# johannah/drqv2

Hardware: NVIDIA B200
Metric: DrQ-v2 updates/sec at batch 256 (higher is better)
Workload: dtype bf16

## Files before the change

drqv2_b200/_bf16.py:

```python
from __future__ import annotations

import ctypes as C

import torch

from . import _lib
from ._lib import (GEMM_KK, GEMM_KMN, GEMM_MNMN, PLB, REPR_DIM, TB_ACT, TB_W, TEPI_F32, TEPI_MASK_BF16,
                   TEPI_RELU_BF16, TEPI_TRUNK_DGRAD, TEPI_TRUNK_WGRAD, WB_SLACK, call)

F32, BF = 4, 2


def _stream():
    return torch.cuda.current_stream().cuda_stream


def _ceil(n, m):
    return (n + m - 1) // m * m


def splitk_for(ctas_per_split, K=REPR_DIM, target_blocks=148):
    s0 = max(1, min(target_blocks // max(1, ctas_per_split), K // 128))
    chunk = -(-K // s0)
    chunk = -(-chunk // 128) * 128
# ... 439 lines not shown
                     ws.metrics.data_ptr() + F32 * 6, xA.ptr(), xA.units, Fd, 0)])
    if split_q:
        twin_q_layers(agent, bw, bw.x, 1, 1, B)
        beside.join()
        twin_q_heads(agent, bw, 2, B)
    else:
        twin_q_fwd(agent, bw, bw.x, 2, B)
    q = bw.q4.data_ptr()
    c1, c2, dc1, dc2 = bw.c1, bw.c2, bw.dc1, bw.dc2
    w0, w2, xC = st.q0, st.q2, bw.x
    U, HS = c1.units, c1.stride
    call("drq_q_head_bwd_loss_bf16", 1, q, q + F32 * 2 * B, ws.reward.data_ptr(), ws.discount.data_ptr(),
         ws.target_q.data_ptr(), ws.metrics.data_ptr(), c2.ptr(), U, HS, pc("Q1.4.weight"), dc2.ptr(),
         gc("Q1.4.weight"), gc("Q1.4.bias"), B, H, qs_f, s)
    with beside:
        gemm(dc2.ptr(), U, c1.ptr(), U, GEMM_MNMN, gc("Q1.2.weight"), H, H, H, B, TEPI_F32, batch=2,
             strides=_strides((HS, HS, qs_f, 0, 0)), bn=128)
    gemm(dc2.ptr(), U, w2.ptr(), w2.units, GEMM_KMN, dc1.ptr(), U, B, H, H, TEPI_MASK_BF16, mask=c1.ptr(), units_mask=U,
         batch=2, strides=_strides((HS, w2.stride, HS, 0, HS)))
    with beside:
        gemm(dc1.ptr(), U, xC.ptr(0), xC.units, GEMM_MNMN, gc("Q1.0.weight"), Fd + A, H, Fd + A, B, TEPI_F32, batch=2,
             strides=_strides((HS, 0, qs_f, 0, 0)))
    PS = B * (Fd + A)
    gemm(dc1.ptr(), U, w0.ptr(), w0.units, GEMM_KMN, bw.dxf.data_ptr(), Fd + A, B, Fd, H, TEPI_F32, batch=2,
         splitk=bw.SX, strides=_strides((HS, w0.stride, PS, 0, 0), split=2 * PS))
    call("drq_ln_tanh_bwd", bw.dxf.data_ptr(), Fd + A, ws.xC.data_ptr(), Fd + A, ws.xhatC.data_ptr(),
         ws.rstdC.data_ptr(), pc("trunk.1.weight"), ws.dz.data_ptr(), None, None,
         bw.dz.ptr(), bw.dz.units, B, Fd, 2 * bw.SX, PS, s)
    with beside:
        gemm(bw.dz.ptr(), bw.dz.units, feat.ptr(), feat.units, GEMM_MNMN, gc("trunk.0.weight"), REPR_DIM, Fd, REPR_DIM, B,
             TEPI_TRUNK_WGRAD, bn=128)
        colsum_multi([ColsumJob(dc2.ptr(0), U, gc("Q1.2.bias"), B, H, 1, 0), ColsumJob(dc2.ptr(1), U, gc("Q2.2.bias"), B, H, 1, 0),
                      ColsumJob(dc1.ptr(0), U, gc("Q1.0.bias"), B, H, 1, 0), ColsumJob(dc1.ptr(1), U, gc("Q2.0.bias"), B, H, 1, 0),
                      ColsumJob(ws.dz.data_ptr(), Fd, gc("trunk.0.bias"), B, Fd, 0, 0),
                      ColsumJob(ws.dz.data_ptr() + F32 * B * Fd, Fd, gc("trunk.1.weight"), B, Fd, 0, 0, ws.xhatC.data_ptr()),
                      ColsumJob(ws.dz.data_ptr() + F32 * B * Fd, Fd, gc("trunk.1.bias"), B, Fd, 0, 0)])
    d = [t.data_ptr() for t in bw.dpre]
    acts = [t.data_ptr() for t in bw.acts]
    ge = lambda k: agent._g("encoder", k)
    if not encoder_grad:
        beside.join()
        agent._sync_grads("critic")
        st.step_critic()
        return
    gemm(bw.dz.ptr(), bw.dz.units, st.trunk_ptr(st.CRITIC), st.trunk.units, GEMM_KMN, d[3], bw.cs_d, B, REPR_DIM, Fd,
         TEPI_TRUNK_DGRAD, mask=feat.ptr(), units_mask=feat.units, bn=128)
    def encoder_backward():
        s2 = _stream()
# ... 209 lines not shown
```

drqv2_b200/_lib.py:

```python
from __future__ import annotations

import ctypes as C
import os
import pathlib

_HERE = pathlib.Path(__file__).resolve().parent
LIB_PATH = _HERE / "csrc" / "libdrqv2_b200.so"

P = C.c_void_p
I = C.c_int
L = C.c_int64
U = C.c_uint64
F = C.c_float

SIGNATURES = {
    "drq_ring_gather_nstep": [P, P, P, P, L, I, I, I, P, P, I, I, F, P, P, P, P, P, P],
    "drq_ring_sample": [P, P, I, U, P, P, P, I, P],
    "drq_rng_update_draws": [U, P, I, P, P, P, P, I, I, P],
    "drq_ring_sample_step": [P, P, I, U, P, P, P, I, P],
    "drq_update_prologue": [P, I, P, P, U, P, I, P, P, P, P, I, I, P],
    "drq_update_prologue_ring": [P, I, P, P, U, P, I, P, P, P, P, I, I, P, P, P, P, P],
    "drq_update_prologue_ring_part": [P, I, P, P, U, P, I, P, P, P, P, I, I, P, P, P, P, I, P],
    "drq_conv1_fwd_bf16_ring": [P, I, P, P, P, I, I, P],
    "drq_conv1_wgrad_bf16_ring": [P, I, P, P, P, P, P, I, I, P],
    "drq_rng_normal_f32": [U, P, P, I, P],
    "drq_counter_advance": [P, P],
    "drq_scalars_fetch": [P, I, P, P, P],
    "drq_random_shift_f32": [P, P, P, I, I, I, I, I, P],
    "drq_conv1_fwd_f32": [P, P, P, P, P, I, I, I, P],
    "drq_conv1_wgrad_f32": [P, P, P, P, P, P, I, I, I, P],
    "drq_conv3x3_fwd_f32": [P, P, P, P, I, I, I, P],
    "drq_conv3x3_dgrad_f32": [P, P, P, P, I, I, P],
    "drq_conv3x3_wgrad_f32": [P, P, P, P, P, I, I, P],
    "drq_pack_conv_w_bf16": [P, P, P, P],
    "drq_conv3x3_fwd_bf16": [P, P, P, P, I, I, I, L, I, I, P],
    "drq_conv3x3_dgrad_bf16": [P, P, P, I, P, I, I, P],
    "drq_conv3x3_wgrad_bf16": [P, I, P, P, P, P, I, I, P],
    "drq_pack_conv1_w_bf16": [P, P, P, I, P],
    "drq_conv1_fwd_bf16": [P, P, P, P, I, I, I, P],
    "drq_conv1_wgrad_bf16": [P, P, P, P, P, P, I, I, I, P],
    "drq_gemm_bf16": [P, I, P, I, I, P, L, I, P, P, I, I, I, I, I, I, I, I, P, I, I, P],
    "drq_set_pdl": [I],
    "drq_set_sm_limit": [I],
    "drq_set_gemm_small": [I],
    "drq_set_conv4x1": [I],
    "drq_set_conv1_planes": [I],
    "drq_debug_gemm_stamps": [P],
    "drq_debug_opt_min_blocks": [I],
    "drq_debug_conv_stamps": [P],
    "drq_debug_trap_note": [P],
    "drq_debug_force_timeout": [P],
    "drq_debug_conv4x1_stamps": [P],
    "drq_debug_conv1_stamps": [P],
    "drq_pack_multi": [P, I, P],
    "drq_conv_wgrad_reduce_multi": [P, I, P],
    "drq_colsum_multi": [P, I, P],
    "drq_pack_linear_tb": [P, P, I, I, P],
    "drq_pack_trunk_tb": [P, P, I, P],
    "drq_pack_features_tb": [P, P, I, P],
    "drq_gemm_f32": [P, L, L, P, L, L, P, L, P, P, L, I, I, I, I, I, I, L, L, L, L, L, I, P],
    "drq_colsum_f32": [P, L, P, I, I, I, L, L, P],
    "drq_ln_tanh_fwd": [P, I, L, P, P, P, P, L, P, P, P, L, I, I, F, P],
    "drq_ln_tanh_fwd_multi": [P, I, I, I, F, P],
    "drq_ln_tanh_bwd": [P, L, P, L, P, P, P, P, P, P, P, L, I, I, I, L, P],
    "drq_actor_sample": [P, P, P, F, P, L, P, P, P, L, I, I, I, P],
    "drq_policy_head_fwd_bf16": [P, L, P, P, P, I, I, I, P, I, P, F, P, P],
    "drq_actor_sample_bwd": [P, L, P, P, P, L, I, I, I, L, P],
# ... 35 lines not shown


def lib():
    global _lib
    if _lib is None:
        if not LIB_PATH.exists():
            raise ImportError(
                f"{LIB_PATH} is missing: build the CUDA extension first (make -C {LIB_PATH.parent}). "
                "drqv2_b200 has no CPU or PyTorch fallback.")
        h = C.CDLL(str(LIB_PATH))
        for name, args in SIGNATURES.items():
            fn = getattr(h, name)
            fn.argtypes, fn.restype = args, I
        for name, (res, args) in SPECIAL.items():
            fn = getattr(h, name)
            fn.argtypes, fn.restype = args, res
        if h.drq_abi_version() != 1:
            raise ImportError("libdrqv2_b200.so ABI version mismatch")
        h.drq_set_pdl(int(os.environ.get("DRQV2_B200_PDL", "0")))
        if os.environ.get("DRQV2_B200_OPT_MINB"):
            h.drq_debug_opt_min_blocks(int(os.environ["DRQV2_B200_OPT_MINB"]))
        if os.environ.get("DRQV2_B200_CONV4X1"):
            h.drq_set_conv4x1(int(os.environ["DRQV2_B200_CONV4X1"]))
        if os.environ.get("DRQV2_B200_CONV1_PLANES"):
            h.drq_set_conv1_planes(int(os.environ["DRQV2_B200_CONV1_PLANES"]))
        _lib = h
    return _lib


def exported_symbols():
    return list(SIGNATURES) + list(SPECIAL)


def call(name, *args):
    rc = getattr(lib(), name)(*args)
    if rc != 0:
        raise DrqError(f"{name} failed ({rc}): {lib().drq_last_error().decode()}")


def ptr(t):
    return None if t is None else t.data_ptr()
```

drqv2_b200/csrc/common.cuh:

```cuda
#pragma once
#include <cuda_runtime.h>
#include <stdint.h>

#include "../../include/drqv2_b200.h"

namespace drq {

void set_error(const char* fmt, ...);

int check_launch(const char* what);

int ensure_smem(const void* kernel, size_t bytes, const char* what);

inline cudaStream_t as_stream(void* s) { return reinterpret_cast<cudaStream_t>(s); }

void* tensor_map_encoder();

extern int g_pdl;
extern int g_pdl_once;
extern int g_sm_limit;
inline int sm_budget() { return g_sm_limit; }
__device__ __forceinline__ void pdl_trigger() {
#ifdef DRQ_PDL_ENTRY_TRIGGER
    asm volatile("griddepcontrol.launch_dependents;" ::: "memory");
#endif
}
__device__ __forceinline__ void pdl_release() { asm volatile("griddepcontrol.launch_dependents;" ::: "memory"); }
__device__ __forceinline__ void pdl_wait() { asm volatile("griddepcontrol.wait;" ::: "memory"); }

template <typename... P, typename... A>
inline void launch_k(void (*kernel)(P...), dim3 grid, dim3 block, size_t smem, cudaStream_t stream, A&&... args) {
    cudaLaunchConfig_t cfg{};
    cfg.gridDim = grid; cfg.blockDim = block; cfg.dynamicSmemBytes = smem; cfg.stream = stream;
    cudaLaunchAttribute attr[1];
    attr[0].id = cudaLaunchAttributeProgrammaticStreamSerialization;
    attr[0].val.programmaticStreamSerializationAllowed = 1;
    cfg.attrs = attr; cfg.numAttrs = (g_pdl == 1 || (g_pdl == 2 && g_pdl_once)) ? 1 : 0;
    g_pdl_once = 0;
    cudaLaunchKernelEx(&cfg, kernel, static_cast<P>(args)...);
}

constexpr int kImg = DRQ_IMG;
constexpr int kPW = DRQ_PW;
constexpr int kPlane = DRQ_PLANE;
constexpr int kCh = DRQ_CONV_CH;

__device__ __forceinline__ int clampi(int v, int lo, int hi) { return v < lo ? lo : (v > hi ? hi : v); }

__device__ __forceinline__ float warp_sum(float v) {
#pragma unroll
    for (int o = 16; o > 0; o >>= 1) v += __shfl_xor_sync(0xffffffffu, v, o);
    return v;
}

struct Philox {
    static constexpr uint32_t kM0 = 0xD2511F53u, kM1 = 0xCD9E8D57u;
    static constexpr uint32_t kW0 = 0x9E3779B9u, kW1 = 0xBB67AE85u;
    __host__ __device__ static inline void round(uint32_t (&c)[4], uint32_t k0, uint32_t k1) {
        uint64_t p0 = (uint64_t)kM0 * c[0], p1 = (uint64_t)kM1 * c[2];
        uint32_t h0 = (uint32_t)(p0 >> 32), l0 = (uint32_t)p0;
        uint32_t h1 = (uint32_t)(p1 >> 32), l1 = (uint32_t)p1;
        uint32_t n0 = h1 ^ c[1] ^ k0, n2 = h0 ^ c[3] ^ k1;
// ... 26 lines not shown
```

drqv2_b200/csrc/gemm_tc.cu:

```cuda
#include "pack.cuh"

namespace drq {

DRQ_TRAP_NOTE_HOOK(trap_note_gemm)

using namespace tc;

constexpr int GT_BM = 128, GT_THREADS = 192;
constexpr int RA = DRQ_TB_ACT, RW = DRQ_TB_W;
constexpr int MODE_KK = DRQ_GEMM_KK, MODE_KMN = DRQ_GEMM_KMN, MODE_MNMN = DRQ_GEMM_MNMN;

struct GemmTcArgs {
    const __nv_bfloat16* A; int units_a;
    const __nv_bfloat16* B; int units_b;
    int M, N, K;
    int batch_inner; long long bs[11];
    int splitk, k_chunk, nz;
    int grid3d;
    int accumulate;
    float* Cf; __nv_bfloat16* Cb; long long ldc;
    int n_store;
    const float* bias;
    const __nv_bfloat16* mask; int units_mask;
    long long* stamps;
};

static long long* g_stamps = nullptr;
#ifdef DRQ_STAMPS
#define GT_STAMP(i) do { if (g.stamps && (blockIdx.x | blockIdx.y | blockIdx.z) == 0) g.stamps[i] = clock64(); } while (0)
#else
#define GT_STAMP(i) do { } while (0)
#endif

template <int MODE, int BN, int EPI, int SMALL = 0>
struct GemmCfg {
    static constexpr int BK = MODE == MODE_MNMN ? RA : 64;
    static constexpr int A_BYTES = MODE == MODE_MNMN ? 16 * RA * 16 : 8 * RA * 16;
    static constexpr int B_BYTES = MODE == MODE_KK ? 8 * BN * 16 : (MODE == MODE_KMN ? (BN / 8) * RW * 16 : (BN / 8) * RA * 16);
    static constexpr int STAGE = A_BYTES + B_BYTES;
    static constexpr bool XPOSE = EPI == DRQ_TEPI_F32 || EPI == DRQ_TEPI_TRUNK_WGRAD;
    static constexpr int XP_FLOATS = EPI == DRQ_TEPI_TRUNK_WGRAD ? 32 * (BN + 1) : (XPOSE ? 32 * 33 : 0);
    static constexpr int EPI_BYTES = 2 * BN * 4 + 4 * XP_FLOATS * 4;
    static constexpr int BUDGET = 196 * 1024 - EPI_BYTES;
    static constexpr int STAGES = SMALL ? 2 : (BUDGET / STAGE > 6 ? 6 : BUDGET / STAGE);
    static constexpr int ACC = 2;
    static constexpr int B_COPIES = (MODE == MODE_KK && BN == 128) ? 2 : 1;
    static constexpr size_t SMEM = (size_t)STAGES * STAGE + EPI_BYTES + (2 * STAGES + 2 * ACC) * 8 + 16;
};

struct TileInfo {
    int m0, n0, k_begin, k_end;
    long long off_a, off_b, off_c, off_bias, off_mask;
};
template <int BN>
__device__ __forceinline__ TileInfo tile_info(const GemmTcArgs& g, int t, int nt, int mt) {
    TileInfo ti;
    int in, im, z;
    if (g.grid3d) {
        in = blockIdx.x; im = blockIdx.y; z = blockIdx.z;
    } else {
        in = t; im = 0; z = 0;
        if (nt > 1) { const int rest = t / nt; in = t - rest * nt; t = rest; } else { in = 0; }
        if (mt > 1) { z = t / mt; im = t - z * mt; } else { z = t; }
    }
    ti.m0 = im * GT_BM; ti.n0 = in * BN;
    int zs = 0, zb = z;
    ti.k_begin = 0; ti.k_end = g.K;
    if (g.splitk > 1) {
        zb = z / g.splitk; zs = z - zb * g.splitk;
        ti.k_begin = zs * g.k_chunk;
        ti.k_end = min(g.K, ti.k_begin + g.k_chunk);
    }
    int zi = zb, zo = 0;
    if (zb >= g.batch_inner) { zo = zb / g.batch_inner; zi = zb - zo * g.batch_inner; }
    ti.off_a = zi * g.bs[0] + zo * g.bs[5];
    ti.off_b = zi * g.bs[1] + zo * g.bs[6];
    ti.off_c = zi * g.bs[2] + zo * g.bs[7] + zs * g.bs[10];
    ti.off_bias = zi * g.bs[3] + zo * g.bs[8];
    ti.off_mask = zi * g.bs[4] + zo * g.bs[9];
    return ti;
}

template <int MODE, int BN, int EPI, int SMALL = 0>
__global__ void __launch_bounds__(GT_THREADS, 1) gemm_tc_kernel(const GemmTcArgs g) {
    using Cfg = GemmCfg<MODE, BN, EPI, SMALL>;
    extern __shared__ __align__(128) uint8_t smem[];
    constexpr int STAGES = Cfg::STAGES, STAGE = Cfg::STAGE, A_BYTES = Cfg::A_BYTES, BK = Cfg::BK, ACC = Cfg::ACC;
    float* bias_s = reinterpret_cast<float*>(smem + STAGES * STAGE);
    float* xpose_s = bias_s + 2 * BN;
    uint64_t* bars = reinterpret_cast<uint64_t*>(smem + STAGES * STAGE + Cfg::EPI_BYTES);
    uint64_t* full = bars;
    uint64_t* empty = bars + STAGES;
    uint64_t* tfull = bars + 2 * STAGES;
    uint64_t* tempty = tfull + ACC;
    uint32_t* tmem_slot = reinterpret_cast<uint32_t*>(tempty + ACC);

    const int tid = threadIdx.x, warp = tid >> 5, lane = tid & 31;
    pdl_trigger();
    if (tid == 0) GT_STAMP(0);
    const int nt = (g.N + BN - 1) / BN, mt = (g.M + GT_BM - 1) / GT_BM;
    const int total_tiles = g.grid3d ? 1 : nt * mt * g.nz;
    const int t_first = g.grid3d ? 0 : blockIdx.x, t_step = g.grid3d ? 1 : gridDim.x;
    if (warp == 0) {
        if (lane == 0) {
            for (int i = 0; i < STAGES; ++i) { mbar_init(full + i, 1 + Cfg::B_COPIES); mbar_init(empty + i, 1); }
            for (int i = 0; i < ACC; ++i) { mbar_init(tfull + i, 1); mbar_init(tempty + i, 4); }
            fence_barrier_init();
        }
        __syncwarp();
        asm volatile("bar.arrive 2, 192;" ::: "memory");
    } else {
        if (warp == 1) {
            tmem_alloc(tmem_slot, ACC * BN);
            tmem_relinquish();
        }
        tc_fence_before();
        asm volatile("bar.sync 2, 192;" ::: "memory");
        tc_fence_after();
    }
    pdl_wait();
    const uint32_t tmem_base = warp == 0 ? 0u : *tmem_slot;
    if (tid == 0) GT_STAMP(1);

    if (warp == 0) {
        if (lane < 1 + Cfg::B_COPIES) {
            int stage = 0; uint32_t phase = 0;
#pragma unroll 1
            for (int t = t_first; t < total_tiles; t += t_step) {
                const TileInfo ti = tile_info<BN>(g, t, nt, mt);
                const int m0 = ti.m0, n0 = ti.n0, k_begin = ti.k_begin, k_end = ti.k_end;
                const int nk = (k_end - k_begin + BK - 1) / BK;
                const __nv_bfloat16* src;
                long long kstep;
                uint32_t bytes = 0;
                uint32_t unit_bytes = 0;
                int units_left = 0;
                if (lane == 0) {
                    if (MODE == MODE_MNMN) {
                        src = g.A + ti.off_a + ((long long)(k_begin / RA) * g.units_a + m0 / 8) * RA * 8;
                        kstep = (long long)g.units_a * RA * 8;
                        bytes = min(16, g.units_a - m0 / 8) * RA * 16;
                    } else {
// ... 2 lines not shown
                        unit_bytes = RA * 16; units_left = (k_end - k_begin + 15) / 16 * 2;
                    }
                } else {
                    if (MODE == MODE_KK) {
                        src = g.B + ti.off_b + ((long long)(n0 / RW + lane - 1) * g.units_b + k_begin / 8) * RW * 8;
                        kstep = 8ll * RW * 8;
                        unit_bytes = RW * 16; units_left = (k_end - k_begin + 15) / 16 * 2;
                    } else if (MODE == MODE_KMN) {
                        src = g.B + ti.off_b + ((long long)(k_begin / RW) * g.units_b + n0 / 8) * RW * 8;
                        kstep = (long long)g.units_b * RW * 8;
                        bytes = min(BN / 8, g.units_b - n0 / 8) * RW * 16;
                    } else {
                        src = g.B + ti.off_b + ((long long)(k_begin / RA) * g.units_b + n0 / 8) * RA * 8;
                        kstep = (long long)g.units_b * RA * 8;
                        bytes = min(BN / 8, g.units_b - n0 / 8) * RA * 16;
                    }
                }
                const uint32_t dst_off = lane == 0 ? 0 : A_BYTES + (lane - 1) * (8 * RW * 16);
#pragma unroll 1
                for (int kb = 0; kb < nk; ++kb) {
                    const uint32_t nbytes = unit_bytes ? min(8, units_left - kb * 8) * unit_bytes : bytes;
                    mbar_wait(empty + stage, phase ^ 1);
                    mbar_arrive_expect_tx(full + stage, nbytes);
                    bulk_g2s(smem + stage * STAGE + dst_off, src, nbytes, full + stage);
                    src += kstep;
                    if (++stage == STAGES) { stage = 0; phase ^= 1; }
                }
            }
        }
        pdl_release();
        if (lane == 0) GT_STAMP(3);
    } else if (warp == 1) {
        constexpr uint32_t idesc = make_idesc_bf16(GT_BM, BN / Cfg::B_COPIES, MODE == MODE_MNMN, MODE != MODE_KK);
        int stage = 0; uint32_t phase = 0; int acc = 0; uint32_t acc_phase = 0;
#pragma unroll 1
        for (int t = t_first; t < total_tiles; t += t_step) {
            const TileInfo ti = tile_info<BN>(g, t, nt, mt);
            const int nk = (ti.k_end - ti.k_begin + BK - 1) / BK;
            mbar_wait(tempty + acc, acc_phase ^ 1);
            const uint32_t d_tmem = tmem_base + acc * BN;
#pragma unroll 1
            for (int kb = 0; kb < nk; ++kb) {
                mbar_wait(full + stage, phase);
                tc_fence_after();
                if (lane == 0 && kb == 0) GT_STAMP(4);
                if (lane == 0 && kb == nk - 1) GT_STAMP(5);
                if (elect_one()) {
                    const int ksteps = min(BK / 16, (ti.k_end - ti.k_begin - kb * BK + 15) / 16);
                    const uint32_t a_addr = smem_u32(smem + stage * STAGE), b_addr = a_addr + A_BYTES;
#pragma unroll 1
                    for (int ks = 0; ks < ksteps; ++ks) {
                        const uint64_t da = MODE == MODE_MNMN ? make_smem_desc(a_addr + ks * 256, 128, RA * 16)
                                                              : make_smem_desc(a_addr + ks * 2 * RA * 16, RA * 16, 128);
                        const uint64_t db = MODE == MODE_KK ? make_smem_desc(b_addr + ks * 2 * RW * 16, RW * 16, 128)
                                           : MODE == MODE_KMN ? make_smem_desc(b_addr + ks * 256, 128, RW * 16)
                                                              : make_smem_desc(b_addr + ks * 256, 128, RA * 16);
                        umma_bf16(d_tmem, da, db, idesc, (kb | ks) ? 1u : 0u);
                        if (Cfg::B_COPIES == 2)
                            umma_bf16(d_tmem + 64, da, make_smem_desc(b_addr + 8 * RW * 16 + ks * 2 * RW * 16, RW * 16, 128), idesc,
                                      (kb | ks) ? 1u : 0u);
                    }
                    umma_commit(empty + stage);
                    if (kb == nk - 1) umma_commit(tfull + acc);
                }
                __syncwarp();
                if (++stage == STAGES) { stage = 0; phase ^= 1; }
            }
            if (++acc == ACC) { acc = 0; acc_phase ^= 1; }
        }
    } else {
        const int q = warp & 3;
        const int et = tid - 64;
        constexpr bool TB_OUT = EPI == DRQ_TEPI_RELU_BF16 || EPI == DRQ_TEPI_MASK_BF16;
        constexpr bool MASKED = EPI == DRQ_TEPI_MASK_BF16 || EPI == DRQ_TEPI_TRUNK_DGRAD;
        float* xp = xpose_s + q * Cfg::XP_FLOATS;
        int acc = 0; uint32_t acc_phase = 0; int it = 0;
#pragma unroll 1
        for (int t = t_first; t < total_tiles; t += t_step, ++it) {
            const TileInfo ti = tile_info<BN>(g, t, nt, mt);
            const int m0 = ti.m0, n0 = ti.n0;
            const long long off_c = ti.off_c;
            const int m = m0 + q * 32 + lane;
            const long long mblk = m / RA, mrow = m % RA;
            const float* bias = g.bias ? g.bias + ti.off_bias : nullptr;
            const __nv_bfloat16* mask = g.mask ? g.mask + ti.off_mask : nullptr;
// ... 27 lines not shown
                }
                tc_fence_before();
                __syncwarp();
                if (lane == 0) mbar_arrive(tempty + acc);
                if (m0 + q * 32 < g.M) {
                    const int px = lane & 15, rsel = lane >> 4;
                    const int u = n0 / 8 + px;
                    const int cu = u / 1225, yx = u - cu * 1225;
                    const bool col_ok = n0 + px * 8 < g.N;
                    float* cbase = g.Cf + off_c + (long long)(cu * 8) * 1225 + yx;
                    const int rows = min(32, g.M - (m0 + q * 32));
#pragma unroll 1
                    for (int ch = 0; ch < 8; ++ch) {
                        float vals[16];
#pragma unroll
                        for (int rp = 0; rp < 16; ++rp) vals[rp] = xp[(rp * 2 + rsel) * XP + px * 8 + ch];
                        float* cb = cbase + (long long)(m0 + q * 32 + rsel) * g.ldc + ch * 1225;
#pragma unroll
                        for (int rp = 0; rp < 16; ++rp)
                            if (rp * 2 + rsel < rows && col_ok) cb[(long long)(rp * 2) * g.ldc] = vals[rp];
                    }
                    __syncwarp();
                }
            } else {
#pragma unroll
                for (int c0 = 0; c0 < BN; c0 += 32) {
                    const int nb = n0 + c0;
                    if (nb >= (TB_OUT ? g.n_store : g.N)) break;
                    float v[32];
                    tmem_ld_32x32(t_acc + c0, v);
                    if (EPI == DRQ_TEPI_F32) {
                        __syncwarp();
#pragma unroll
                        for (int j = 0; j < 32; ++j) xp[lane * 33 + j] = v[j] + bs[c0 + j];
                        __syncwarp();
                        const int n = nb + lane;
                        const int rows = min(32, g.M - (m0 + q * 32));
                        float* cbase = g.Cf + off_c + (long long)(m0 + q * 32) * g.ldc + n;
                        if (n < g.N) {
#pragma unroll 4
                            for (int r = 0; r < rows; ++r) {
                                float x = xp[r * 33 + lane];
                                if (g.accumulate) x += cbase[r * g.ldc];
                                cbase[r * g.ldc] = x;
                            }
                        }
// ... 33 lines not shown
                                        hi = n + 1 < g.N ? fmaxf(hi + bs[c0 + 8 * c + 2 * j + 1], 0.f) : 0.f;
                                    } else {
                                        lo = (n < g.N && bf16_lo(mw[j]) > 0.f) ? lo : 0.f;
                                        hi = (n + 1 < g.N && bf16_hi(mw[j]) > 0.f) ? hi : 0.f;
                                    }
                                    pk[j] = pack_bf16x2(lo, hi);
                                }
                                *reinterpret_cast<uint4*>(g.Cb + off_c + ((mblk * g.ldc + n8 / 8) * RA + mrow) * 8) =
                                    make_uint4(pk[0], pk[1], pk[2], pk[3]);
                            }
                        }
                    }
                }
                tc_fence_before();
                __syncwarp();
                if (lane == 0) mbar_arrive(tempty + acc);
            }
            if (++acc == ACC) { acc = 0; acc_phase ^= 1; }
        }
    }
    if (tid == 64) GT_STAMP(7);
    tc_fence_before();
    __syncthreads();
    if (warp == 1) tmem_dealloc(tmem_base, ACC * BN);
    if (tid == 0) GT_STAMP(8);
}

static int g_gemm_small = 0;

template <int MODE, int BN, int EPI, int SMALL = 0>
static int launch_gemm_tc(GemmTcArgs& g, int batch, cudaStream_t s) {
    using Cfg = GemmCfg<MODE, BN, EPI, SMALL>;
    if (int rc = ensure_smem((const void*)gemm_tc_kernel<MODE, BN, EPI, SMALL>, Cfg::SMEM, "gemm_bf16")) return rc;
    g.nz = g.splitk * batch;
    const int nt = (g.N + BN - 1) / BN, mt = (g.M + GT_BM - 1) / GT_BM;
    const int tiles = nt * mt * g.nz;
    const int sms = drq_device_sm_count();
    g.grid3d = tiles <= sms ? 1 : 0;
    launch_k(gemm_tc_kernel<MODE, BN, EPI, SMALL>, g.grid3d ? dim3(nt, mt, g.nz) : dim3(sms), GT_THREADS, Cfg::SMEM, s, g);
    return check_launch("gemm_tc_kernel");
}

__global__ void __launch_bounds__(256)
pack_linear_tb_kernel(const float* __restrict__ w, __nv_bfloat16* __restrict__ out, int rows, int cols, int units) {
    pdl_trigger();
    pdl_wait();
    pack_linear_tb_block(w, out, rows, cols, units, blockIdx.x, blockIdx.y, threadIdx.x);
}

__global__ void __launch_bounds__(256)
pack_trunk_tb_kernel(const float* __restrict__ w, __nv_bfloat16* __restrict__ out, int rows) {
    pdl_trigger();
    pdl_wait();
    __shared__ float tile[32][33];
    pack_trunk_tb_block(w, out, rows, blockIdx.x, blockIdx.y, threadIdx.x, tile);
}

__global__ void __launch_bounds__(256)
pack_features_tb_kernel(const float* __restrict__ f, __nv_bfloat16* __restrict__ out, int rows) {
    pdl_trigger();
    pdl_wait();
    __shared__ float tile[32][33];
    pack_trunk_tb_block<DRQ_TB_ACT>(f, out, rows, blockIdx.x, blockIdx.y, threadIdx.x, tile);
// ... 27 lines not shown
        DRQ_REQUIRE(mode == MODE_KK ? units_b * 8 >= K : units_b * 8 >= N, "gemm_bf16: B units too small");
    }
    GemmTcArgs g{};
    g.A = reinterpret_cast<const __nv_bfloat16*>(A); g.units_a = units_a;
    g.B = reinterpret_cast<const __nv_bfloat16*>(B); g.units_b = units_b;
    g.M = M; g.N = N; g.K = K;
    g.batch_inner = batch_inner;
    for (int i = 0; i < 11; ++i) g.bs[i] = strides ? strides[i] : 0;
    for (int i = 0; i < 10; ++i)
        if (i % 5 == 0 || i % 5 == 1 || i % 5 == 4)
            DRQ_REQUIRE(g.bs[i] % 8 == 0, "gemm_bf16: bf16 batch strides must keep 16-byte alignment");
    g.splitk = splitk; g.k_chunk = K;
    if (splitk > 1) {
        int chunk = (K + splitk - 1) / splitk;
        chunk = (chunk + 127) / 128 * 128;
        g.k_chunk = chunk;
        DRQ_REQUIRE((long long)chunk * (splitk - 1) < K, "gemm_bf16: splitk %d leaves empty chunks for K=%d", splitk, K);
    }
    g.accumulate = accumulate;
    g.Cf = reinterpret_cast<float*>(C); g.Cb = reinterpret_cast<__nv_bfloat16*>(C); g.ldc = ldc;
    g.n_store = n_store > N ? n_store : N;
    g.bias = splitk > 1 ? nullptr : bias;
    g.mask = reinterpret_cast<const __nv_bfloat16*>(mask); g.units_mask = units_mask;
    g.stamps = g_stamps;
    cudaStream_t s = as_stream(stream);
#define GT_CASE(MODE_, BN_, EPI_) \
    if (mode == MODE_ && bn == BN_ && epilogue == EPI_) return launch_gemm_tc<MODE_, BN_, EPI_>(g, batch, s);
#define GT_SMALL(MODE_, BN_, EPI_) \
    if (g_gemm_small && mode == MODE_ && bn == BN_ && epilogue == EPI_) return launch_gemm_tc<MODE_, BN_, EPI_, 1>(g, batch, s);
    GT_SMALL(MODE_KK, 64, DRQ_TEPI_F32)
    GT_SMALL(MODE_KK, 64, DRQ_TEPI_RELU_BF16)
    GT_SMALL(MODE_KMN, 64, DRQ_TEPI_F32)
    GT_SMALL(MODE_KMN, 64, DRQ_TEPI_MASK_BF16)
    GT_CASE(MODE_KK, 64, DRQ_TEPI_F32)
    GT_CASE(MODE_KK, 64, DRQ_TEPI_RELU_BF16)
    GT_CASE(MODE_KK, 128, DRQ_TEPI_F32)
    GT_CASE(MODE_KK, 128, DRQ_TEPI_RELU_BF16)
    GT_CASE(MODE_KMN, 64, DRQ_TEPI_F32)
    GT_CASE(MODE_KMN, 64, DRQ_TEPI_MASK_BF16)
    GT_CASE(MODE_KMN, 128, DRQ_TEPI_MASK_BF16)
    GT_CASE(MODE_KMN, 128, DRQ_TEPI_TRUNK_DGRAD)
    GT_CASE(MODE_MNMN, 64, DRQ_TEPI_F32)
    GT_CASE(MODE_MNMN, 128, DRQ_TEPI_F32)
    GT_CASE(MODE_MNMN, 128, DRQ_TEPI_TRUNK_WGRAD)
#undef GT_CASE
#undef GT_SMALL
    set_error("gemm_bf16: no kernel for mode %d, bn %d, epilogue %d", mode, bn, epilogue);
    return DRQ_ERR_INVALID;
}

int drq_set_gemm_small(int on) { g_gemm_small = on ? 1 : 0; return DRQ_OK; }

int drq_debug_gemm_stamps(int64_t* buf) { g_stamps = reinterpret_cast<long long*>(buf); return DRQ_OK; }

int drq_pack_linear_tb(const float* w, uint16_t* out, int rows, int cols, void* stream) {
    DRQ_REQUIRE(w && out && rows > 0 && cols > 0, "pack_linear_tb: bad args");
    const int units = (cols + 15) / 16 * 2;
    const int rpad = (rows + RW - 1) / RW * RW;
    launch_k(pack_linear_tb_kernel, dim3((rpad + 255) / 256, units), 256, 0, as_stream(stream), 
        w, reinterpret_cast<__nv_bfloat16*>(out), rows, cols, units);
    return check_launch("pack_linear_tb_kernel");
}

int drq_pack_trunk_tb(const float* w, uint16_t* out, int rows, void* stream) {
    DRQ_REQUIRE(w && out && rows > 0, "pack_trunk_tb: bad args");
    const int rpad = (rows + RW - 1) / RW * RW;
    launch_k(pack_trunk_tb_kernel, dim3((1225 + 31) / 32, rpad), 256, 0, as_stream(stream), 
        w, reinterpret_cast<__nv_bfloat16*>(out), rows);
    return check_launch("pack_trunk_tb_kernel");
}

int drq_pack_features_tb(const float* feat, uint16_t* out, int rows, void* stream) {
    DRQ_REQUIRE(feat && out && rows > 0, "pack_features_tb: bad args");
    DRQ_REQUIRE(((uintptr_t)out % 16) == 0, "pack_features_tb: output must be 16-byte aligned");
// ... 8 lines not shown
```

drqv2_b200/csrc/tc_common.cuh:

```cuda
#pragma once
#include <cuda_bf16.h>

#include "common.cuh"

namespace drq {
namespace tc {

__device__ __forceinline__ uint32_t smem_u32(const void* p) {
    return static_cast<uint32_t>(__cvta_generic_to_shared(p));
}

static __device__ unsigned int* volatile g_trap_note = nullptr;
#define DRQ_TRAP_NOTE_HOOK(name)                                                                               \
    int name(unsigned int* p) { return cudaMemcpyToSymbol(drq::tc::g_trap_note, &p, sizeof(p)) == cudaSuccess ? 0 : 1; }

__device__ __forceinline__ void mbar_init(uint64_t* bar, uint32_t count) {
    asm volatile("mbarrier.init.shared::cta.b64 [%0], %1;" ::"r"(smem_u32(bar)), "r"(count));
}
__device__ __forceinline__ void fence_barrier_init() {
    asm volatile("fence.mbarrier_init.release.cluster;" ::: "memory");
}
__device__ __forceinline__ void fence_proxy_async() {
    asm volatile("fence.proxy.async.shared::cta;" ::: "memory");
}
// ... 42 lines not shown
            "mbarrier.try_wait.parity.shared::cta.b64 p, [%1], %2;\n\t"
            "selp.u32 %0, 1, 0, p;\n\t}"
            : "=r"(done)
            : "r"(addr), "r"(parity)
            : "memory");
        if (done) return;
        __nanosleep(SLEEP_NS);
    }
    if (g_trap_note) {
        g_trap_note[1] = blockDim.x; g_trap_note[2] = threadIdx.x; g_trap_note[3] = addr; g_trap_note[4] = parity; g_trap_note[5] = blockIdx.x;
        __threadfence_system();
        g_trap_note[0] = 2u;
        __threadfence_system();
    }
    __trap();
}

__device__ __forceinline__ void bulk_g2s(void* smem_dst, const void* gmem_src, uint32_t bytes, uint64_t* bar) {
    asm volatile("cp.async.bulk.shared::cluster.global.mbarrier::complete_tx::bytes [%0], [%1], %2, [%3];"
                 :
                 : "r"(smem_u32(smem_dst)), "l"(gmem_src), "r"(bytes), "r"(smem_u32(bar))
                 : "memory");
}

__device__ __forceinline__ bool elect_one() {
    uint32_t pred = 0;
    asm volatile(
        "{\n\t.reg .b32 rx;\n\t.reg .pred px;\n\t"
        "elect.sync rx|px, 0xFFFFFFFF;\n\t"
        "selp.u32 %0, 1, 0, px;\n\t}"
        : "=r"(pred));
    return pred != 0;
}
__device__ __forceinline__ void tmem_alloc(uint32_t* smem_dst, uint32_t ncols) {
    asm volatile("tcgen05.alloc.cta_group::1.sync.aligned.shared::cta.b32 [%0], %1;" ::"r"(smem_u32(smem_dst)),
                 "r"(ncols)
                 : "memory");
}
__device__ __forceinline__ void tmem_relinquish() {
    asm volatile("tcgen05.relinquish_alloc_permit.cta_group::1.sync.aligned;" ::: "memory");
}
__device__ __forceinline__ void tmem_dealloc(uint32_t taddr, uint32_t ncols) {
    asm volatile("tcgen05.dealloc.cta_group::1.sync.aligned.b32 %0, %1;" ::"r"(taddr), "r"(ncols) : "memory");
}
__device__ __forceinline__ void tc_fence_before() { asm volatile("tcgen05.fence::before_thread_sync;" ::: "memory"); }
__device__ __forceinline__ void tc_fence_after() { asm volatile("tcgen05.fence::after_thread_sync;" ::: "memory"); }
__device__ __forceinline__ void tmem_wait_ld() { asm volatile("tcgen05.wait::ld.sync.aligned;" ::: "memory"); }

__device__ __forceinline__ void umma_commit(uint64_t* bar) {
    asm volatile("tcgen05.commit.cta_group::1.mbarrier::arrive::one.shared::cluster.b64 [%0];" ::"r"(smem_u32(bar))
                 : "memory");
}

__device__ __forceinline__ void umma_bf16(uint32_t tmem_d, uint64_t desc_a, uint64_t desc_b, uint32_t idesc,
                                          uint32_t accumulate) {
    asm volatile(
        "{\n\t.reg .pred p;\n\t"
        "setp.ne.b32 p, %4, 0;\n\t"
        "tcgen05.mma.cta_group::1.kind::f16 [%0], %1, %2, %3, p;\n\t}"
        :
        : "r"(tmem_d), "l"(desc_a), "l"(desc_b), "r"(idesc), "r"(accumulate)
        : "memory");
}

__host__ __device__ constexpr uint32_t make_idesc_bf16(int M, int N, bool a_mn_major, bool b_mn_major) {
    return (1u << 4)
           | (1u << 7)
           | (1u << 10)
           | ((a_mn_major ? 1u : 0u) << 15)
           | ((b_mn_major ? 1u : 0u) << 16)
           | ((uint32_t)(N >> 3) << 17) | ((uint32_t)(M >> 4) << 24);
}

// ... 45 lines not shown
```

include/drqv2_b200.h:

```cpp
#ifndef DRQV2_B200_H
#define DRQV2_B200_H

#include <stdint.h>

#ifdef __cplusplus
extern "C" {
#endif

#define DRQ_SCAL_SLOT 32
#define DRQ_ABI_VERSION 1

#define DRQ_OK 0
#define DRQ_ERR_INVALID 1
#define DRQ_ERR_CUDA 2

#define DRQ_IMG 84
#define DRQ_PW 41
#define DRQ_PLANE 1696
#define DRQ_CONV_CH 32
#define DRQ_REPR_DIM 39200

#define DRQ_PLB 1776
#define DRQ_GUARD 88
#define DRQ_WB_SLACK 128

#define DRQ_EPI_NONE 0
#define DRQ_EPI_RELU 1
#define DRQ_EPI_MASK 2
#define DRQ_EPI_MASK_WIDE 3

int drq_abi_version(void);
const char* drq_last_error(void);
int drq_device_sm_count(void);
int drq_set_pdl(int on);
int drq_set_sm_limit(int sms);
int drq_set_gemm_small(int on);
int drq_set_conv4x1(int mode);
int drq_set_conv1_planes(int on);


int drq_ring_gather_nstep(const uint8_t* frames, const float* action, const float* reward,
                          const float* discount, int64_t capacity, int frame_c, int stack, int A,
                          const int32_t* ep_start, const int32_t* idx, int B, int nstep,
                          float gamma, uint8_t* obs_out, uint8_t* next_obs_out,
                          float* action_out, float* reward_out, float* discount_out,
                          void* stream);

int drq_ring_sample(const int32_t* ep_table, const int32_t* n_episodes, int nstep, uint64_t seed,
                    const uint64_t* counter, int32_t* ep_start_out, int32_t* idx_out, int B,
                    void* stream);


int drq_rng_update_draws(uint64_t seed, const uint64_t* counter, int pad, int32_t* shift_obs,
                         int32_t* shift_next, float* eps_critic, float* eps_actor, int B, int A,
                         void* stream);
int drq_rng_normal_f32(uint64_t seed, const uint64_t* counter, float* out, int n, void* stream);
int drq_counter_advance(uint64_t* counter, void* stream);

int drq_scalars_fetch(const float* ring, int slots, uint64_t* cursor, float* out, void* stream);
// ... 222 lines not shown
```

Measured before the change: 2097.

## Add cluster multicast GEMM, staged trunk dgrad epilogue, small-GEMM for critic dxf

Adds an optional thread-block-cluster path for BN=64 GEMMs that multicasts the A operand tiles across the CTAs of a cluster, with cluster-wide empty-barrier commits. It also adds a staged trunk-dgrad epilogue that masks the accumulator, transposes it through shared memory and issues coalesced 16-byte stores into the padded plane layout, and this path is enabled by default. Separately, the critic input-gradient GEMM is switched to the SMALL configuration (two stages). Cluster mode defaults to 1, so the multicast path stays dormant unless an environment variable enables it, while the other two changes run by default. The risks are extra shared memory for the staging buffer and fewer pipeline stages on that GEMM.

```diff
diff --git a/drqv2_b200/_bf16.py b/drqv2_b200/_bf16.py
--- a/drqv2_b200/_bf16.py
+++ b/drqv2_b200/_bf16.py
@@ -485,8 +485,12 @@
         gemm(dc1.ptr(), U, xC.ptr(0), xC.units, GEMM_MNMN, gc("Q1.0.weight"), Fd + A, H, Fd + A, B, TEPI_F32, batch=2,
              strides=_strides((HS, 0, qs_f, 0, 0)))
     PS = B * (Fd + A)
-    gemm(dc1.ptr(), U, w0.ptr(), w0.units, GEMM_KMN, bw.dxf.data_ptr(), Fd + A, B, Fd, H, TEPI_F32, batch=2,
-         splitk=bw.SX, strides=_strides((HS, w0.stride, PS, 0, 0), split=2 * PS))
+    call("drq_set_gemm_small", 1)
+    try:
+        gemm(dc1.ptr(), U, w0.ptr(), w0.units, GEMM_KMN, bw.dxf.data_ptr(), Fd + A, B, Fd, H, TEPI_F32, batch=2,
+             splitk=bw.SX, strides=_strides((HS, w0.stride, PS, 0, 0), split=2 * PS))
+    finally:
+        call("drq_set_gemm_small", 0)
     call("drq_ln_tanh_bwd", bw.dxf.data_ptr(), Fd + A, ws.xC.data_ptr(), Fd + A, ws.xhatC.data_ptr(),
          ws.rstdC.data_ptr(), pc("trunk.1.weight"), ws.dz.data_ptr(), None, None,
          bw.dz.ptr(), bw.dz.units, B, Fd, 2 * bw.SX, PS, s)
diff --git a/drqv2_b200/_lib.py b/drqv2_b200/_lib.py
--- a/drqv2_b200/_lib.py
+++ b/drqv2_b200/_lib.py
@@ -43,6 +43,8 @@
     "drq_set_pdl": [I],
     "drq_set_sm_limit": [I],
     "drq_set_gemm_small": [I],
+    "drq_set_gemm_cluster": [I],
+    "drq_set_trunk_dgrad_staged": [I],
     "drq_set_conv4x1": [I],
     "drq_set_conv1_planes": [I],
     "drq_debug_gemm_stamps": [P],
@@ -124,6 +126,10 @@
             h.drq_debug_opt_min_blocks(int(os.environ["DRQV2_B200_OPT_MINB"]))
         if os.environ.get("DRQV2_B200_CONV4X1"):
             h.drq_set_conv4x1(int(os.environ["DRQV2_B200_CONV4X1"]))
+        if os.environ.get("DRQV2_B200_GEMM_CLUSTER"):
+            h.drq_set_gemm_cluster(int(os.environ["DRQV2_B200_GEMM_CLUSTER"]))
+        if os.environ.get("DRQV2_B200_DGRAD_STAGED"):
+            h.drq_set_trunk_dgrad_staged(int(os.environ["DRQV2_B200_DGRAD_STAGED"]))
         if os.environ.get("DRQV2_B200_CONV1_PLANES"):
             h.drq_set_conv1_planes(int(os.environ["DRQV2_B200_CONV1_PLANES"]))
         _lib = h
diff --git a/drqv2_b200/csrc/common.cuh b/drqv2_b200/csrc/common.cuh
--- a/drqv2_b200/csrc/common.cuh
+++ b/drqv2_b200/csrc/common.cuh
@@ -29,15 +29,28 @@
 __device__ __forceinline__ void pdl_wait() { asm volatile("griddepcontrol.wait;" ::: "memory"); }
 
 template <typename... P, typename... A>
-inline void launch_k(void (*kernel)(P...), dim3 grid, dim3 block, size_t smem, cudaStream_t stream, A&&... args) {
+inline void launch_k_cluster(int cluster_x, void (*kernel)(P...), dim3 grid, dim3 block, size_t smem, cudaStream_t stream,
+                             A&&... args) {
     cudaLaunchConfig_t cfg{};
     cfg.gridDim = grid; cfg.blockDim = block; cfg.dynamicSmemBytes = smem; cfg.stream = stream;
-    cudaLaunchAttribute attr[1];
-    attr[0].id = cudaLaunchAttributeProgrammaticStreamSerialization;
-    attr[0].val.programmaticStreamSerializationAllowed = 1;
-    cfg.attrs = attr; cfg.numAttrs = (g_pdl == 1 || (g_pdl == 2 && g_pdl_once)) ? 1 : 0;
+    cudaLaunchAttribute attr[2];
+    unsigned n = 0;
+    if (g_pdl == 1 || (g_pdl == 2 && g_pdl_once)) {
+        attr[n].id = cudaLaunchAttributeProgrammaticStreamSerialization;
+        attr[n++].val.programmaticStreamSerializationAllowed = 1;
+    }
+    if (cluster_x > 1) {
+        attr[n].id = cudaLaunchAttributeClusterDimension;
+        attr[n].val.clusterDim.x = cluster_x; attr[n].val.clusterDim.y = 1; attr[n++].val.clusterDim.z = 1;
+    }
+    cfg.attrs = attr; cfg.numAttrs = n;
     g_pdl_once = 0;
     cudaLaunchKernelEx(&cfg, kernel, static_cast<P>(args)...);
+}
+
+template <typename... P, typename... A>
+inline void launch_k(void (*kernel)(P...), dim3 grid, dim3 block, size_t smem, cudaStream_t stream, A&&... args) {
+    launch_k_cluster(1, kernel, grid, block, smem, stream, static_cast<A&&>(args)...);
 }
 
 constexpr int kImg = DRQ_IMG;
diff --git a/drqv2_b200/csrc/gemm_tc.cu b/drqv2_b200/csrc/gemm_tc.cu
--- a/drqv2_b200/csrc/gemm_tc.cu
+++ b/drqv2_b200/csrc/gemm_tc.cu
@@ -22,6 +22,7 @@
     int n_store;
     const float* bias;
     const __nv_bfloat16* mask; int units_mask;
+    int dgrad_staged;
     long long* stamps;
 };
 
@@ -38,8 +39,9 @@
     static constexpr int A_BYTES = MODE == MODE_MNMN ? 16 * RA * 16 : 8 * RA * 16;
     static constexpr int B_BYTES = MODE == MODE_KK ? 8 * BN * 16 : (MODE == MODE_KMN ? (BN / 8) * RW * 16 : (BN / 8) * RA * 16);
     static constexpr int STAGE = A_BYTES + B_BYTES;
-    static constexpr bool XPOSE = EPI == DRQ_TEPI_F32 || EPI == DRQ_TEPI_TRUNK_WGRAD;
-    static constexpr int XP_FLOATS = EPI == DRQ_TEPI_TRUNK_WGRAD ? 32 * (BN + 1) : (XPOSE ? 32 * 33 : 0);
+    static constexpr bool XPOSE = EPI == DRQ_TEPI_F32 || EPI == DRQ_TEPI_TRUNK_WGRAD || EPI == DRQ_TEPI_TRUNK_DGRAD;
+    static constexpr int XP_FLOATS = EPI == DRQ_TEPI_TRUNK_WGRAD ? 32 * (BN + 1)
+                                   : EPI == DRQ_TEPI_TRUNK_DGRAD ? 32 * (BN / 8 + 1) * 4 : (XPOSE ? 32 * 33 : 0);
     static constexpr int EPI_BYTES = 2 * BN * 4 + 4 * XP_FLOATS * 4;
     static constexpr int BUDGET = 196 * 1024 - EPI_BYTES;
     static constexpr int STAGES = SMALL ? 2 : (BUDGET / STAGE > 6 ? 6 : BUDGET / STAGE);
@@ -81,8 +83,9 @@
     return ti;
 }
 
-template <int MODE, int BN, int EPI, int SMALL = 0>
+template <int MODE, int BN, int EPI, int SMALL = 0, int CL = 1>
 __global__ void __launch_bounds__(GT_THREADS, 1) gemm_tc_kernel(const GemmTcArgs g) {
+    static_assert(CL == 1 || (MODE != MODE_MNMN && 8 % CL == 0), "multicast of K-major A tiles only");
     using Cfg = GemmCfg<MODE, BN, EPI, SMALL>;
     extern __shared__ __align__(128) uint8_t smem[];
     constexpr int STAGES = Cfg::STAGES, STAGE = Cfg::STAGE, A_BYTES = Cfg::A_BYTES, BK = Cfg::BK, ACC = Cfg::ACC;
@@ -103,7 +106,7 @@
     const int t_first = g.grid3d ? 0 : blockIdx.x, t_step = g.grid3d ? 1 : gridDim.x;
     if (warp == 0) {
         if (lane == 0) {
-            for (int i = 0; i < STAGES; ++i) { mbar_init(full + i, 1 + Cfg::B_COPIES); mbar_init(empty + i, 1); }
+            for (int i = 0; i < STAGES; ++i) { mbar_init(full + i, 1 + Cfg::B_COPIES); mbar_init(empty + i, CL); }
             for (int i = 0; i < ACC; ++i) { mbar_init(tfull + i, 1); mbar_init(tempty + i, 4); }
             fence_barrier_init();
         }
@@ -118,6 +121,7 @@
         asm volatile("bar.sync 2, 192;" ::: "memory");
         tc_fence_after();
     }
+    if (CL > 1) cluster_sync();
     pdl_wait();
     const uint32_t tmem_base = warp == 0 ? 0u : *tmem_slot;
     if (tid == 0) GT_STAMP(1);
@@ -166,8 +170,22 @@
                     const uint32_t nbytes = unit_bytes ? min(8, units_left - kb * 8) * unit_bytes : bytes;
                     mbar_wait(empty + stage, phase ^ 1);
                     mbar_arrive_expect_tx(full + stage, nbytes);
-                    bulk_g2s(smem + stage * STAGE + dst_off, src, nbytes, full + stage);
+                    if (CL > 1 && lane == 0) {
+                        const uint32_t u0 = cluster_ctarank() * (8 / CL), units = nbytes / unit_bytes;
+                        if (u0 < units)
+                            bulk_g2s_multicast(smem + stage * STAGE + u0 * unit_bytes, src + u0 * RA * 8,
+                                               min(8u / CL, units - u0) * unit_bytes, full + stage, (1u << CL) - 1);
+                    } else {
+                        bulk_g2s(smem + stage * STAGE + dst_off, src, nbytes, full + stage);
+                    }
                     src += kstep;
+                    if (++stage == STAGES) { stage = 0; phase ^= 1; }
+                }
+            }
+            if (CL > 1 && lane == 0) {
+#pragma unroll 1
+                for (int i = 0; i < STAGES; ++i) {
+                    mbar_wait(empty + stage, phase ^ 1);
                     if (++stage == STAGES) { stage = 0; phase ^= 1; }
                 }
             }
@@ -204,7 +222,8 @@
                             umma_bf16(d_tmem + 64, da, make_smem_desc(b_addr + 8 * RW * 16 + ks * 2 * RW * 16, RW * 16, 128), idesc,
                                       (kb | ks) ? 1u : 0u);
                     }
-                    umma_commit(empty + stage);
+                    if (CL > 1) umma_commit_multicast(empty + stage, (1u << CL) - 1);
+                    else umma_commit(empty + stage);
                     if (kb == nk - 1) umma_commit(tfull + acc);
                 }
                 __syncwarp();
@@ -278,6 +297,43 @@
                     }
                     __syncwarp();
                 }
+            } else if (EPI == DRQ_TEPI_TRUNK_DGRAD && g.dgrad_staged) {
+                constexpr int UN = BN / 8, XS = UN + 1;
+                uint4* xs = reinterpret_cast<uint4*>(xp);
+#pragma unroll
+                for (int c0 = 0; c0 < BN; c0 += 32) {
+                    if (n0 + c0 >= g.N) break;
+                    float v[32];
+                    tmem_ld_32x32(t_acc + c0, v);
+#pragma unroll
+                    for (int c = 0; c < 4; ++c) {
+                        const uint4 mv = mk[c0 / 8 + c];
+                        const uint32_t mw[4] = {mv.x, mv.y, mv.z, mv.w};
+                        uint32_t pk[4];
+#pragma unroll
+                        for (int j = 0; j < 4; ++j)
+                            pk[j] = pack_bf16x2(bf16_lo(mw[j]) > 0.f ? v[8 * c + 2 * j] : 0.f,
+                                                bf16_hi(mw[j]) > 0.f ? v[8 * c + 2 * j + 1] : 0.f);
+                        xs[lane * XS + c0 / 8 + c] = make_uint4(pk[0], pk[1], pk[2], pk[3]);
+                    }
+                }
+                tc_fence_before();
+                __syncwarp();
+                if (lane == 0) mbar_arrive(tempty + acc);
+                static_assert(EPI != DRQ_TEPI_TRUNK_DGRAD || UN == 16, "two images of 16 units per store instruction");
+                const int px = lane & 15, rsel = lane >> 4;
+                const int u = n0 / 8 + px;
+                const int cu = u / 1225, yx = u - cu * 1225;
+                const int yy = yx / 35, xx = yx - yy * 35;
+                const int mb = m0 + q * 32;
+                if (u * 8 < g.N) {
+                    __nv_bfloat16* cb = g.Cb + (cu * g.ldc + DRQ_GUARD + yy * DRQ_PW + xx) * 8;
+                    const int rows = min(32, g.M - mb);
+#pragma unroll 4
+                    for (int r = rsel; r < rows; r += 2)
+                        *reinterpret_cast<uint4*>(cb + (long long)(mb + r) * DRQ_PLB * 8) = xs[r * XS + px];
+                }
+                __syncwarp();
             } else {
 #pragma unroll
                 for (int c0 = 0; c0 < BN; c0 += 32) {
@@ -357,23 +413,36 @@
     if (tid == 64) GT_STAMP(7);
     tc_fence_before();
     __syncthreads();
+    if (CL > 1) cluster_sync();
     if (warp == 1) tmem_dealloc(tmem_base, ACC * BN);
     if (tid == 0) GT_STAMP(8);
 }
 
 static int g_gemm_small = 0;
-
-template <int MODE, int BN, int EPI, int SMALL = 0>
+static int g_gemm_cluster = 1;
+static int g_dgrad_staged = 1;
+
+template <int MODE, int BN, int EPI, int SMALL = 0, int CL = 1>
 static int launch_gemm_tc(GemmTcArgs& g, int batch, cudaStream_t s) {
-    using Cfg = GemmCfg<MODE, BN, EPI, SMALL>;
-    if (int rc = ensure_smem((const void*)gemm_tc_kernel<MODE, BN, EPI, SMALL>, Cfg::SMEM, "gemm_bf16")) return rc;
     g.nz = g.splitk * batch;
     const int nt = (g.N + BN - 1) / BN, mt = (g.M + GT_BM - 1) / GT_BM;
     const int tiles = nt * mt * g.nz;
     const int sms = drq_device_sm_count();
     g.grid3d = tiles <= sms ? 1 : 0;
-    launch_k(gemm_tc_kernel<MODE, BN, EPI, SMALL>, g.grid3d ? dim3(nt, mt, g.nz) : dim3(sms), GT_THREADS, Cfg::SMEM, s, g);
+    if constexpr (CL > 1)
+        if (!(g.grid3d && nt % CL == 0)) return launch_gemm_tc<MODE, BN, EPI, SMALL, 1>(g, batch, s);
+    using Cfg = GemmCfg<MODE, BN, EPI, SMALL>;
+    if (int rc = ensure_smem((const void*)gemm_tc_kernel<MODE, BN, EPI, SMALL, CL>, Cfg::SMEM, "gemm_bf16")) return rc;
+    launch_k_cluster(CL, gemm_tc_kernel<MODE, BN, EPI, SMALL, CL>, g.grid3d ? dim3(nt, mt, g.nz) : dim3(sms), GT_THREADS,
+                     Cfg::SMEM, s, g);
     return check_launch("gemm_tc_kernel");
+}
+
+template <int MODE, int EPI>
+static int launch_gemm_tc_cl(GemmTcArgs& g, int batch, cudaStream_t s) {
+    if (g_gemm_cluster == 4) return launch_gemm_tc<MODE, 64, EPI, 0, 4>(g, batch, s);
+    if (g_gemm_cluster == 2) return launch_gemm_tc<MODE, 64, EPI, 0, 2>(g, batch, s);
+    return launch_gemm_tc<MODE, 64, EPI>(g, batch, s);
 }
 
 __global__ void __launch_bounds__(256)
@@ -447,34 +516,50 @@
     g.n_store = n_store > N ? n_store : N;
     g.bias = splitk > 1 ? nullptr : bias;
     g.mask = reinterpret_cast<const __nv_bfloat16*>(mask); g.units_mask = units_mask;
+    g.dgrad_staged = g_dgrad_staged;
     g.stamps = g_stamps;
     cudaStream_t s = as_stream(stream);
 #define GT_CASE(MODE_, BN_, EPI_) \
     if (mode == MODE_ && bn == BN_ && epilogue == EPI_) return launch_gemm_tc<MODE_, BN_, EPI_>(g, batch, s);
+#define GT_CLUSTER(MODE_, EPI_) \
+    if (mode == MODE_ && bn == 64 && epilogue == EPI_) return launch_gemm_tc_cl<MODE_, EPI_>(g, batch, s);
 #define GT_SMALL(MODE_, BN_, EPI_) \
     if (g_gemm_small && mode == MODE_ && bn == BN_ && epilogue == EPI_) return launch_gemm_tc<MODE_, BN_, EPI_, 1>(g, batch, s);
     GT_SMALL(MODE_KK, 64, DRQ_TEPI_F32)
     GT_SMALL(MODE_KK, 64, DRQ_TEPI_RELU_BF16)
     GT_SMALL(MODE_KMN, 64, DRQ_TEPI_F32)
     GT_SMALL(MODE_KMN, 64, DRQ_TEPI_MASK_BF16)
-    GT_CASE(MODE_KK, 64, DRQ_TEPI_F32)
-    GT_CASE(MODE_KK, 64, DRQ_TEPI_RELU_BF16)
+    GT_CLUSTER(MODE_KK, DRQ_TEPI_F32)
+    GT_CLUSTER(MODE_KK, DRQ_TEPI_RELU_BF16)
     GT_CASE(MODE_KK, 128, DRQ_TEPI_F32)
     GT_CASE(MODE_KK, 128, DRQ_TEPI_RELU_BF16)
-    GT_CASE(MODE_KMN, 64, DRQ_TEPI_F32)
-    GT_CASE(MODE_KMN, 64, DRQ_TEPI_MASK_BF16)
+    GT_CLUSTER(MODE_KMN, DRQ_TEPI_F32)
+    GT_CLUSTER(MODE_KMN, DRQ_TEPI_MASK_BF16)
     GT_CASE(MODE_KMN, 128, DRQ_TEPI_MASK_BF16)
     GT_CASE(MODE_KMN, 128, DRQ_TEPI_TRUNK_DGRAD)
     GT_CASE(MODE_MNMN, 64, DRQ_TEPI_F32)
     GT_CASE(MODE_MNMN, 128, DRQ_TEPI_F32)
     GT_CASE(MODE_MNMN, 128, DRQ_TEPI_TRUNK_WGRAD)
 #undef GT_CASE
+#undef GT_CLUSTER
 #undef GT_SMALL
     set_error("gemm_bf16: no kernel for mode %d, bn %d, epilogue %d", mode, bn, epilogue);
     return DRQ_ERR_INVALID;
 }
 
 int drq_set_gemm_small(int on) { g_gemm_small = on ? 1 : 0; return DRQ_OK; }
+
+int drq_set_gemm_cluster(int ctas) {
+    const int prev = g_gemm_cluster;
+    if (ctas == 1 || ctas == 2 || ctas == 4) g_gemm_cluster = ctas;
+    return prev;
+}
+
+int drq_set_trunk_dgrad_staged(int on) {
+    const int prev = g_dgrad_staged;
+    if (on == 0 || on == 1) g_dgrad_staged = on;
+    return prev;
+}
 
 int drq_debug_gemm_stamps(int64_t* buf) { g_stamps = reinterpret_cast<long long*>(buf); return DRQ_OK; }
 
diff --git a/drqv2_b200/csrc/tc_common.cuh b/drqv2_b200/csrc/tc_common.cuh
--- a/drqv2_b200/csrc/tc_common.cuh
+++ b/drqv2_b200/csrc/tc_common.cuh
@@ -88,6 +88,22 @@
                  : "r"(smem_u32(smem_dst)), "l"(gmem_src), "r"(bytes), "r"(smem_u32(bar))
                  : "memory");
 }
+__device__ __forceinline__ void bulk_g2s_multicast(void* smem_dst, const void* gmem_src, uint32_t bytes, uint64_t* bar,
+                                                   uint16_t cta_mask) {
+    asm volatile("cp.async.bulk.shared::cluster.global.mbarrier::complete_tx::bytes.multicast::cluster [%0], [%1], %2, [%3], %4;"
+                 :
+                 : "r"(smem_u32(smem_dst)), "l"(gmem_src), "r"(bytes), "r"(smem_u32(bar)), "h"(cta_mask)
+                 : "memory");
+}
+
+__device__ __forceinline__ uint32_t cluster_ctarank() {
+    uint32_t r;
+    asm volatile("mov.u32 %0, %%cluster_ctarank;" : "=r"(r));
+    return r;
+}
+__device__ __forceinline__ void cluster_sync() {
+    asm volatile("barrier.cluster.arrive.release.aligned;\n\tbarrier.cluster.wait.acquire.aligned;" ::: "memory");
+}
 
 __device__ __forceinline__ bool elect_one() {
     uint32_t pred = 0;
@@ -115,6 +131,11 @@
 
 __device__ __forceinline__ void umma_commit(uint64_t* bar) {
     asm volatile("tcgen05.commit.cta_group::1.mbarrier::arrive::one.shared::cluster.b64 [%0];" ::"r"(smem_u32(bar))
+                 : "memory");
+}
+__device__ __forceinline__ void umma_commit_multicast(uint64_t* bar, uint16_t cta_mask) {
+    asm volatile("tcgen05.commit.cta_group::1.mbarrier::arrive::one.shared::cluster.multicast::cluster.b64 [%0], %1;"
+                 ::"r"(smem_u32(bar)), "h"(cta_mask)
                  : "memory");
 }
 
diff --git a/include/drqv2_b200.h b/include/drqv2_b200.h
--- a/include/drqv2_b200.h
+++ b/include/drqv2_b200.h
@@ -35,6 +35,8 @@
 int drq_set_pdl(int on);
 int drq_set_sm_limit(int sms);
 int drq_set_gemm_small(int on);
+int drq_set_gemm_cluster(int ctas);
+int drq_set_trunk_dgrad_staged(int on);
 int drq_set_conv4x1(int mode);
 int drq_set_conv1_planes(int on);
 
```

Result: no change. 2109 (median of 6 runs) (+0.6%).
